# DakeQQ/Audio-Denoiser-ONNX

Measured on AMD Instinct MI355X. Metric: audio_seconds_per_second (GTCRN 16 kHz, batch=256 x 1 s chunks; RTF = 1/value), higher is better.
Workload: dtype f32; 1 GPU; GTCRN 16 kHz, batch=256 x 1 s chunks, fp32, int16 PCM in/out resident in HBM (BASELINE.json configs[1]); chunks_per_gpu=256, chunks_total=256, ranks=1, chunk_samples=16000, out_samples=15872, weights=seeded reference-architecture GTCRN (tests/golden/gtcrn_seed0.adew), stitch_all_gather=False

## Files before the change

audio_denoiser_onnx_amd/csrc/ade_device.h:

```cpp
#pragma once

#include "ade_internal.h"

namespace ade {
namespace dev {

__device__ __forceinline__ float fast_rcp(float x) { return __builtin_amdgcn_rcpf(x); }
__device__ __forceinline__ float fast_sqrt(float x) { return __builtin_amdgcn_sqrtf(x); }
__device__ __forceinline__ float fast_rsq(float x) { return __builtin_amdgcn_rsqf(x); }
__device__ __forceinline__ float sigmoid_f(float x) { return fast_rcp(1.0f + __expf(-x)); }
__device__ __forceinline__ float tanh_f(float x) {
    return 1.0f - 2.0f * fast_rcp(__expf(2.0f * x) + 1.0f);
}
__device__ __forceinline__ float prelu_f(float x, float a) { return x >= 0.0f ? x : a * x; }
__device__ __forceinline__ double shfl_xor_f64(double v, int mask) {
    union { double d; int i[2]; } u;
    u.d = v;
    u.i[0] = __shfl_xor(u.i[0], mask, 64);
    u.i[1] = __shfl_xor(u.i[1], mask, 64);
    return u.d;
}
__device__ __forceinline__ float prelu_sel(float a) { return a <= 1.0f ? __builtin_inff() : -__builtin_inff(); }
__device__ __forceinline__ float prelu_m(float x, float ax, float sel) { return __builtin_amdgcn_fmed3f(x, ax, sel); }

__device__ __forceinline__ void ld4(const float* p, float* v) {
    const float4 q = *reinterpret_cast<const float4*>(p);
    v[0] = q.x; v[1] = q.y; v[2] = q.z; v[3] = q.w;
}
__device__ __forceinline__ void ld8(const float* p, float* v) { ld4(p, v); ld4(p + 4, v + 4); }
__device__ __forceinline__ void ld16(const float* p, float* v) { ld8(p, v); ld8(p + 8, v + 8); }
__device__ __forceinline__ void st4(float* p, const float* v) {
    *reinterpret_cast<float4*>(p) = make_float4(v[0], v[1], v[2], v[3]);
}
__device__ __forceinline__ void st16(float* p, const float* v) { st4(p, v); st4(p + 4, v + 4); st4(p + 8, v + 8); st4(p + 12, v + 12); }

__device__ __forceinline__ void view_ld8_lo(const View& a, size_t pos, size_t frame, float* v) {
    ld8(a.x + pos * kCh, v);
    if (a.at) {
        float g[4];
        ld4(a.at + frame * 8, g);
#pragma unroll
        for (int i = 0; i < 4; ++i) v[2 * i] *= g[i];
    }
}
__device__ __forceinline__ void view_ld8_hi(const View& a, size_t pos, size_t frame, float* v) {
    ld8(a.x + pos * kCh + 8, v);
    if (a.at) {
        float g[4];
        ld4(a.at + frame * 8 + 4, g);
#pragma unroll
        for (int i = 0; i < 4; ++i) v[2 * i] *= g[i];
    }
}
__device__ __forceinline__ void view_ld16(const View& a, size_t pos, size_t frame, float* v) {
    view_ld8_lo(a, pos, frame, v);
    view_ld8_hi(a, pos, frame, v + 8);
}

template <int CTRL>
__device__ __forceinline__ float dpp_mov(float v) {
    return __int_as_float(__builtin_amdgcn_update_dpp(0, __float_as_int(v), CTRL, 0xF, 0xF, true));
}
template <int K> __device__ __forceinline__ float row_bcast(float v) { return dpp_mov<0x150 + K>(v); }
template <int K> __device__ __forceinline__ float quad_bcast(float v) { return dpp_mov<K * 0x55>(v); }
template <int N> __device__ __forceinline__ float row_ror(float v) { return dpp_mov<0x120 + N>(v); }
template <int N> __device__ __forceinline__ float quad_rot(float v) {
    return dpp_mov<((N) & 3) | (((N + 1) & 3) << 2) | (((N + 2) & 3) << 4) | (((N + 3) & 3) << 6)>(v);
}

struct Swapped { float a, b; };
__device__ __forceinline__ Swapped swap16(float v, float s) {
    const auto r = __builtin_amdgcn_permlane16_swap((unsigned)__float_as_int(v), (unsigned)__float_as_int(s), false, false);
    return Swapped{__int_as_float((int)r[0]), __int_as_float((int)r[1])};
}
__device__ __forceinline__ Swapped swap32(float v, float s) {
    const auto r = __builtin_amdgcn_permlane32_swap((unsigned)__float_as_int(v), (unsigned)__float_as_int(s), false, false);
    return Swapped{__int_as_float((int)r[0]), __int_as_float((int)r[1])};
}

template <int LANE> __device__ __forceinline__ float read_lane(float v) {
    return __int_as_float(__builtin_amdgcn_readlane(__float_as_int(v), LANE));
}
constexpr float kLog2e = 1.4426950408889634f;

#if defined(__clang__)
typedef float v4f __attribute__((ext_vector_type(4)));
#else
typedef float v4f __attribute__((vector_size(16)));
#endif
__device__ __forceinline__ v4f mfma16x16x4(float a, float b, v4f c) { return __builtin_amdgcn_mfma_f32_16x16x4f32(a, b, c, 0, 0, 0); }

#if defined(__clang__)
typedef float v2f __attribute__((ext_vector_type(2)));
#else
typedef float v2f __attribute__((vector_size(8)));
#endif
__device__ __forceinline__ v2f mk2(float a, float b) { v2f r; r[0] = a; r[1] = b; return r; }

#if defined(__has_attribute)
#if __has_attribute(address_space)
#define ADE_CONSTANT_AS __attribute__((address_space(4)))
#endif
#endif
#ifndef ADE_CONSTANT_AS
#define ADE_CONSTANT_AS
#endif
#if defined(__AMDGCN__)
#define ADE_KEEP_IN_LOOP(p) asm volatile("" : "+s"(p))
#else
#define ADE_KEEP_IN_LOOP(p) ((void)0)
#endif
#if defined(__AMDGCN__)
#define ADE_KEEP_AFTER(p, tok) asm volatile("" : "+s"(p), "+v"(tok))
#else
#define ADE_KEEP_AFTER(p, tok) ((void)0)
#endif
#if defined(__AMDGCN__)
#define ADE_SCALAR_COPY(dst, src) asm volatile("s_mov_b64 %0, %1" : "=s"(dst) : "s"(src))
#else
#define ADE_SCALAR_COPY(dst, src) ((dst) = (src))
#endif
#if defined(__AMDGCN__)
#define ADE_OPAQUE_V(x) asm volatile("" : "+v"(x))
#else
#define ADE_OPAQUE_V(x) ((void)0)
#endif
template <class T>
__device__ __forceinline__ T cload(const void ADE_CONSTANT_AS* p) {
    static_assert(sizeof(T) % 4 == 0, "dword-sized structs only");
    union U { T v; unsigned w[sizeof(T) / 4]; __device__ U() {} } u;
    const unsigned ADE_CONSTANT_AS* s = (const unsigned ADE_CONSTANT_AS*)p;
#pragma unroll
    for (size_t i = 0; i < sizeof(T) / 4; ++i) u.w[i] = s[i];
    return u.v;
}
typedef const float ADE_CONSTANT_AS* cfptr;
__device__ __forceinline__ cfptr cptr(const float* p) { return (cfptr)p; }

__device__ __forceinline__ void wave_sync() { __builtin_amdgcn_wave_barrier(); }
__device__ __forceinline__ float2 fcmul(float2 a, float2 b) { return make_float2(a.x * b.x - a.y * b.y, a.x * b.y + a.y * b.x); }
__device__ __forceinline__ void fradix4(float2* v) {
    const float2 a0 = make_float2(v[0].x + v[2].x, v[0].y + v[2].y);
    const float2 a1 = make_float2(v[0].x - v[2].x, v[0].y - v[2].y);
    const float2 a2 = make_float2(v[1].x + v[3].x, v[1].y + v[3].y);
    const float2 d = make_float2(v[1].x - v[3].x, v[1].y - v[3].y);
    const float2 a3 = make_float2(d.y, -d.x);
    v[0] = make_float2(a0.x + a2.x, a0.y + a2.y);
    v[1] = make_float2(a1.x + a3.x, a1.y + a3.y);
    v[2] = make_float2(a0.x - a2.x, a0.y - a2.y);
    v[3] = make_float2(a1.x - a3.x, a1.y - a3.y);
}
__device__ __forceinline__ void fft256_inplace(float2* v, float2* buf, int lane, const float2* __restrict__ tw256) {
    fradix4(v);
#pragma unroll
    for (int r = 0; r < 4; ++r) buf[4 * lane + r] = v[r];
    wave_sync();
#pragma unroll
    for (int pass = 1; pass < 4; ++pass) {
        const int Ns = 1 << (2 * pass);
        const int k = lane & (Ns - 1);
        const int tstride = 64 / Ns;
#pragma unroll
        for (int r = 0; r < 4; ++r) v[r] = buf[lane + 64 * r];
#pragma unroll
        for (int r = 1; r < 4; ++r) v[r] = fcmul(v[r], tw256[r * k * tstride]);
        fradix4(v);
        if (pass < 3) {
            wave_sync();
            const int j0 = ((lane - k) << 2) + k;
#pragma unroll
            for (int r = 0; r < 4; ++r) buf[j0 + r * Ns] = v[r];
            wave_sync();
        }
    }
}

__device__ __forceinline__ float4 keep4(bool ok, const float4& v) { return make_float4(ok ? v.x : 0.0f, ok ? v.y : 0.0f, ok ? v.z : 0.0f, ok ? v.w : 0.0f); }
__device__ __attribute__((aligned(16))) static float g_zero4[4] = {0.0f, 0.0f, 0.0f, 0.0f};
__device__ __forceinline__ float4 ld4_or_zero(bool ok, const float* p) { return *reinterpret_cast<const float4*>(ok ? p : g_zero4); }
__device__ __forceinline__ float4 pick4(bool first, const float4& a, const float4& b) {
    return make_float4(first ? a.x : b.x, first ? a.y : b.y, first ? a.z : b.z, first ? a.w : b.w);
}

#if defined(__AMDGCN__)
typedef unsigned ade_v4u __attribute__((ext_vector_type(4)));
__device__ __forceinline__ float4 xld4(const float* base, int float_off) {
    const __amdgpu_buffer_rsrc_t r = __builtin_amdgcn_make_buffer_rsrc(const_cast<float*>(base), 0, 0x7fffffff, 0x00020000);
    const ade_v4u v = __builtin_amdgcn_raw_buffer_load_b128(r, float_off * 4, 0, 16);
    return make_float4(__int_as_float((int)v.x), __int_as_float((int)v.y), __int_as_float((int)v.z), __int_as_float((int)v.w));
}
__device__ __forceinline__ void xst4(float* base, int float_off, const float4& v) {
    const __amdgpu_buffer_rsrc_t r = __builtin_amdgcn_make_buffer_rsrc(base, 0, 0x7fffffff, 0x00020000);
    ade_v4u u;
    u.x = (unsigned)__float_as_int(v.x); u.y = (unsigned)__float_as_int(v.y); u.z = (unsigned)__float_as_int(v.z); u.w = (unsigned)__float_as_int(v.w);
    __builtin_amdgcn_raw_buffer_store_b128(u, r, float_off * 4, 0, 16);
}
__device__ __forceinline__ float xld1(const float* p) { return __hip_atomic_load(p, __ATOMIC_RELAXED, __HIP_MEMORY_SCOPE_AGENT); }
__device__ __forceinline__ void xst1(float* p, float v) { __hip_atomic_store(p, v, __ATOMIC_RELAXED, __HIP_MEMORY_SCOPE_AGENT); }
__device__ __forceinline__ unsigned xflag_load(const unsigned* p) { return __hip_atomic_load(p, __ATOMIC_RELAXED, __HIP_MEMORY_SCOPE_AGENT); }
__device__ __forceinline__ void xflag_store(unsigned* p, unsigned v) { __hip_atomic_store(p, v, __ATOMIC_RELAXED, __HIP_MEMORY_SCOPE_AGENT); }
__device__ __forceinline__ void xdrain() { asm volatile("s_waitcnt vmcnt(0)" ::: "memory"); }
#else
__device__ __forceinline__ float4 xld4(const float* base, int float_off) { return *reinterpret_cast<const float4*>(base + float_off); }
__device__ __forceinline__ void xst4(float* base, int float_off, const float4& v) { *reinterpret_cast<float4*>(base + float_off) = v; }
__device__ __forceinline__ float xld1(const float* p) { return *p; }
__device__ __forceinline__ void xst1(float* p, float v) { *p = v; }
__device__ __forceinline__ unsigned xflag_load(const unsigned* p) { return *(const volatile unsigned*)p; }
__device__ __forceinline__ void xflag_store(unsigned* p, unsigned v) { *(volatile unsigned*)p = v; }
__device__ __forceinline__ void xdrain() {}
#endif
#if defined(__AMDGCN__)
__device__ __forceinline__ int xlimit() {
    const int ADE_CONSTANT_AS* p = (const int ADE_CONSTANT_AS*)__builtin_amdgcn_kernarg_segment_ptr();
    asm volatile("" : "+s"(p));
    return *p;
}
#else
__device__ __forceinline__ int xlimit() { return 20000000; }
#endif
__device__ __forceinline__ int xcode(int flag_index) { return (int)((blockIdx.x + 1u) << 4) | flag_index; }
__device__ __forceinline__ void xwait(unsigned* flag, int* err, int code) {
    if (xflag_load(flag) == 0u) {
        const long long t0 = wall_clock64();
        const int limit = xlimit();
        bool looked = false;
        do {
            __builtin_amdgcn_s_sleep(4);
            const long long dt = wall_clock64() - t0;
            if (dt > (limit >> 4) && !looked) {
                looked = true;
                if (*reinterpret_cast<volatile int*>(err) != 0) return;
            }
            if (dt > limit) {
                volatile int* const e = reinterpret_cast<volatile int*>(err);
                if (*e == 0) *e = code;
                return;
            }
        } while (xflag_load(flag) == 0u);
    }
    xflag_store(flag, 0u);
}

#if defined(__AMDGCN__)
__device__ __forceinline__ unsigned sys_load(const unsigned* p) { return __hip_atomic_load(p, __ATOMIC_RELAXED, __HIP_MEMORY_SCOPE_SYSTEM); }
__device__ __forceinline__ void sys_store(unsigned* p, unsigned v) { __hip_atomic_store(p, v, __ATOMIC_RELAXED, __HIP_MEMORY_SCOPE_SYSTEM); }
__device__ __forceinline__ void sys_acquire() { __builtin_amdgcn_fence(__ATOMIC_ACQUIRE, ""); }
__device__ __forceinline__ void sys_release() { __builtin_amdgcn_fence(__ATOMIC_RELEASE, ""); asm volatile("s_waitcnt vmcnt(0)" ::: "memory"); }
#else
__device__ __forceinline__ unsigned sys_load(const unsigned* p) { return *(const volatile unsigned*)p; }
__device__ __forceinline__ void sys_store(unsigned* p, unsigned v) { *(volatile unsigned*)p = v; }
__device__ __forceinline__ void sys_acquire() {}
__device__ __forceinline__ void sys_release() {}
#endif
__device__ __forceinline__ void wait_rows_in(const unsigned* ready, unsigned epoch, int* err, int code) {
    if (sys_load(ready) != epoch) {
        const long long t0 = wall_clock64();
        const int limit = xlimit();
        do {
            __builtin_amdgcn_s_sleep(8);
            if (wall_clock64() - t0 > limit) {
                volatile int* const e = reinterpret_cast<volatile int*>(err);
                if (*e == 0) *e = code;
                break;
            }
        } while (sys_load(ready) != epoch);
    }
    sys_acquire();
}
__device__ __forceinline__ void signal_rows_out(unsigned* count, unsigned* done, unsigned epoch, unsigned wgs) {
    sys_release();
#if defined(__AMDGCN__)
    const unsigned old = __hip_atomic_fetch_add(count, 1u, __ATOMIC_RELAXED, __HIP_MEMORY_SCOPE_AGENT);
#else
    const unsigned old = (*count)++;
#endif
    if (old + 1u == wgs) {
        xflag_store(count, 0u);
        sys_store(done, epoch);
    }
}

__device__ __forceinline__ void set_prio(int p) {
    if (p == 0) __builtin_amdgcn_s_setprio(0);
    else if (p == 1) __builtin_amdgcn_s_setprio(1);
    else if (p == 2) __builtin_amdgcn_s_setprio(2);
    else __builtin_amdgcn_s_setprio(3);
}

inline dim3 grid1(long long n, int per) { return dim3((unsigned)((n + per - 1) / per)); }

}
}
```

audio_denoiser_onnx_amd/csrc/ade_stage_net.h:

```cpp
#pragma once
#include "ade_device.h"

#include <type_traits>

#ifndef ADE_DP_INTER_MFMA
#define ADE_DP_INTER_MFMA 0
#endif

namespace ade {
namespace stage {

using namespace dev;


template <int NT, int TMAX, int WAVES_PER_SIMD>
struct Geo {
    static constexpr int kThreads = NT;
    static constexpr int kWavesPerSimd = WAVES_PER_SIMD;
    static constexpr int kTmax = TMAX;
    static constexpr int kPmax = TMAX * kFw;
    static constexpr int kPosPerThread = (kPmax + NT - 1) / NT;
    static constexpr int kTileF = NT / 64;
    static constexpr int kProdBase = ((TMAX * (kFw / 3) + 63) / 64) * 64;
    static constexpr bool kLean = NT < 512;
    static_assert(kPosPerThread == 3, "the conv phases are written for three positions per lane");
    static_assert(kProdBase < NT, "the history producers need a wavefront outside the conv lanes");
};
typedef Geo<1024, 64, 4> Geo0;
typedef Geo<512, 32, 4> Geo1;
typedef Geo<256, 16, 4> Geo2;

__device__ __forceinline__ float comp(const float4& v, int c) { return c == 0 ? v.x : (c == 1 ? v.y : (c == 2 ? v.z : v.w)); }

__device__ __forceinline__ void pl_ld8(const float* Xc, int P, int p, int q0, float* v) {
    ld4(Xc + ((size_t)q0 * P + p) * 4, v);
    ld4(Xc + ((size_t)(q0 + 1) * P + p) * 4, v + 4);
}
__device__ __forceinline__ void pl_ld16(const float* Xc, int P, int p, float* v) {
    pl_ld8(Xc, P, p, 0, v);
    pl_ld8(Xc, P, p, 2, v + 8);
}
__device__ __forceinline__ void pl_st16(float* Xc, int P, int p, const float* v) {
#pragma unroll
    for (int q = 0; q < 4; ++q) st4(Xc + ((size_t)q * P + p) * 4, v + 4 * q);
}

template <class G> constexpr size_t gt_smem_bytes() { return (size_t)4 * G::kPmax * 16 + 2 * G::kTmax * 8 * 4; }

#define ADE_REP16(M) M(0) M(1) M(2) M(3) M(4) M(5) M(6) M(7) M(8) M(9) M(10) M(11) M(12) M(13) M(14) M(15)

#define ADE_CLK(i) do { if (clk && chunk == 0 && threadIdx.x == 0) clk[i] = wall_clock64(); } while (0)
#define ADE_CLK_START() ((clk && chunk == 0 && threadIdx.x == 0) ? wall_clock64() : 0)
#define ADE_CLK_ACC(i) do { if (clk && chunk == 0 && threadIdx.x == 0) { const long long n_ = wall_clock64(); clk[i] += n_ - clk_prev; clk_prev = n_; } } while (0)

template <class G>
__device__ __forceinline__ void gtblock_stage(float4* smem, int chunk, const Seg& sg, int blk, const float* __restrict__ a, const float* __restrict__ skip,
                                              const GtConvW& w, float* __restrict__ out, long long* __restrict__ clk,
                                              bool x1_in_lds = false, bool next_x1 = false, const float* __restrict__ next_skip = nullptr, bool store_lo = true,
                                              bool next_full = false) {
    constexpr int kFusedThreads = G::kThreads, kTmaxFused = G::kTmax, kPmax = G::kPmax, kPosPerThread = G::kPosPerThread;
    float4* H = smem;
    float* zt = reinterpret_cast<float*>(smem + 4 * kPmax);
    float* at = zt + kTmaxFused * 8;
    float* GI = reinterpret_cast<float*>(smem + 2 * kPmax);
    float* HS = GI + kTmaxFused * 48;
    const int T = sg.nT;
    const int P = T * kFw;
    const int Ps = sg.T * kFw;
    int tid_ = threadIdx.x;
    if (kFusedThreads == 512 && sg.swap) tid_ ^= (tid_ & 256) >> 1;
    ADE_OPAQUE_V(tid_);
    const int tid = tid_;
    const size_t cbase = (size_t)chunk * kCh * Ps + (size_t)sg.t0 * kFw * 4;
    const float* ac = a + cbase;
    const float* sc = skip ? skip + cbase : nullptr;
    float* oc = out + cbase;
    const cfptr c_pw1_b = cptr(w.pw1_b), c_dw_b = cptr(w.dw_b), c_pw2_b = cptr(w.pw2_b);
    cfptr c_pw1, c_dw, c_pw2;
    ADE_SCALAR_COPY(c_pw1, cptr(w.pw1));
    ADE_SCALAR_COPY(c_dw, cptr(w.dw));
    ADE_SCALAR_COPY(c_pw2, cptr(w.pw2));
    const float pw1_slope = w.pw1_slope, dw_slope = w.dw_slope;
    const float pw1_sel = prelu_sel(pw1_slope), dw_sel = prelu_sel(dw_slope);
    const int dilation = w.dilation;
    ADE_CLK(0);

    if (!x1_in_lds) {
        constexpr int kIt = (kPmax + kFusedThreads - 1) / kFusedThreads;
        float x[kIt][8], y[kIt][8];
#pragma unroll
        for (int i = 0; i < kIt; ++i) {
            const int p = tid + i * kFusedThreads, pc = p < P ? p : P - 1;
            pl_ld8(ac, Ps, pc, 0, x[i]);
            if (sc) pl_ld8(sc, Ps, pc, 0, y[i]);
        }
#pragma unroll
        for (int i = 0; i < kIt; ++i) {
            const int p = tid + i * kFusedThreads;
            if (p >= P) break;
            if (sc) {
#pragma unroll
                for (int k = 0; k < 8; ++k) x[i][k] += y[i][k];
            }
            H[2 * kPmax + p] = make_float4(x[i][0], x[i][1], x[i][2], x[i][3]);
            H[3 * kPmax + p] = make_float4(x[i][4], x[i][5], x[i][6], x[i][7]);
        }
        __syncthreads();
    }
    constexpr int kWaves = kFusedThreads / 64;
    constexpr int kTiles = (kPmax / 16 + kWaves - 1) / kWaves;
    static_assert(kPmax % 16 == 0, "whole tiles");
    const int wave = __builtin_amdgcn_readfirstlane(tid >> 6);
    const int g = (tid >> 4) & 3, jn = tid & 15;
    const float* Hf = reinterpret_cast<const float*>(H);
    const char* const Hb = reinterpret_cast<const char*>(H);
    constexpr int kZ0 = 4 * kPmax * 16;
    constexpr int kPairs = (kTiles + 1) / 2;
    float4 hi[kPairs];
    {
        float wa[2][6];
#pragma unroll
        for (int kk = 0; kk < 6; ++kk) {
            wa[0][kk] = c_pw1[((4 * (kk & 1) + g) * 3 + (kk >> 1)) * 16 + jn];
            wa[1][kk] = c_pw1[((4 * (kk & 1) + g) * 3 + (kk >> 1)) * 16 + (jn ^ 8)];
        }
        v4f cb[2];
#pragma unroll
        for (int r = 0; r < 4; ++r) { cb[0][r] = c_pw1_b[4 * g + r]; cb[1][r] = c_pw1_b[(4 * g + r) ^ 8]; }
#pragma unroll
        for (int it = 0; it < kTiles; ++it) {
            const int od = it & 1;
            const int pu = (it * kWaves + wave) * 16 + jn, pos = pu < P ? pu : P - 1;
            const int f = pos - (pos / kFw) * kFw;
            const bool lok = f != 0, rok = f != kFw - 1;
            const char* xb = Hb + (pos * 4 + g) * 4;
            v4f d = cb[od];
#pragma unroll
            for (int kk = 0; kk < 6; ++kk) {
                const int o = kk >> 1;
                float x = *reinterpret_cast<const float*>(xb + ((2 + (kk & 1)) * kPmax + (o - 1)) * 16);
                if (o == 0) x = lok ? x : 0.0f;
                if (o == 2) x = rok ? x : 0.0f;
                d = mfma16x16x4(wa[od][kk], x, d);
            }
            const v2f d0 = mk2(d[0], d[1]), d1 = mk2(d[2], d[3]);
            const v2f a0 = d0 * mk2(pw1_slope, pw1_slope), a1 = d1 * mk2(pw1_slope, pw1_slope);
            const float4 r4 = make_float4(prelu_m(d0[0], a0[0], pw1_sel), prelu_m(d0[1], a0[1], pw1_sel),
                                          prelu_m(d1[0], a1[0], pw1_sel), prelu_m(d1[1], a1[1], pw1_sel));
            const bool now = (g < 2) != (od != 0);
            if (now && pu < P) H[(g & 1) * kPmax + pu] = r4;
            if (!od) {
                hi[it >> 1] = r4;
            } else {
                hi[it >> 1] = make_float4(now ? hi[it >> 1].x : r4.x, now ? hi[it >> 1].y : r4.y, now ? hi[it >> 1].z : r4.z, now ? hi[it >> 1].w : r4.w);
            }
        }
    }
    __syncthreads();
#pragma unroll
    for (int pr = 0; pr < kPairs; ++pr) {
        const int it = 2 * pr + (g < 2 ? 1 : 0);
        const int pu = (it * kWaves + wave) * 16 + jn;
        if (it < kTiles && pu < P) H[(2 + (g & 1)) * kPmax + pu] = hi[pr];
    }
    if (tid < 12) zt[tid] = 0.0f;
    if (sg.prev && tid == 0) xwait(sg.fi + kXFlagHist + blk, sg.err, xcode(kXFlagHist + blk));
    __syncthreads();
    ADE_CLK(1);

    float4 h1r[kPairs];
    {
        v2f wd[3][3][2];
#pragma unroll
        for (int kt = 0; kt < 3; ++kt)
#pragma unroll
            for (int kf = 0; kf < 3; ++kf) {
                const int o = kt * 48 + kf * 16 + 4 * g;
                wd[kt][kf][0] = mk2(c_dw[o], c_dw[o + 1]);
                wd[kt][kf][1] = mk2(c_dw[o + 2], c_dw[o + 3]);
            }
        const v2f db0 = mk2(c_dw_b[4 * g], c_dw_b[4 * g + 1]), db1 = mk2(c_dw_b[4 * g + 2], c_dw_b[4 * g + 3]);
        const int dstep = dilation * kFw * 16;
        const char* const zp = Hb + kZ0;
        auto dw_taps = [&](v2f& acc0, v2f& acc1, const int tj, const int f, const int prow, const int nkt) {
            const bool lok = f != 0, rok = f != kFw - 1;
            const char* const rb = Hb + ((g * kPmax + prow) * 16 - 16);
#pragma unroll
            for (int kt = 0; kt < 3; ++kt) {
                if (kt >= nkt) continue;
                const int src = tj - (2 - kt) * dilation;
                const bool tv = nkt == 3 ? (kt == 2 ? true : prow >= (2 - kt) * dilation * kFw) : (src >= 0 && src < T);
                const char* const row = tv ? rb - (2 - kt) * dstep : zp;
                const char* const la = lok ? row : zp;
                const char* const ra = rok ? row : zp;
                const float4 x0 = *reinterpret_cast<const float4*>(la);
                const float4 x1 = *reinterpret_cast<const float4*>(row + 16);
                const float4 x2 = *reinterpret_cast<const float4*>(ra + 32);
                acc0 += wd[kt][0][0] * mk2(x0.x, x0.y);
                acc1 += wd[kt][0][1] * mk2(x0.z, x0.w);
                acc0 += wd[kt][1][0] * mk2(x1.x, x1.y);
                acc1 += wd[kt][1][1] * mk2(x1.z, x1.w);
                acc0 += wd[kt][2][0] * mk2(x2.x, x2.y);
                acc1 += wd[kt][2][1] * mk2(x2.z, x2.w);
            }
        };
        float* const xhist_o = sg.xo + blk * kXHistFloats;
        const float* const xhist_i = sg.xi + blk * kXHistFloats;
        const int NP = 2 * dilation * kFw;
        if (sg.next) {
#pragma unroll 1
            for (int pt = wave; pt * 16 < NP; pt += kWaves) {
                const int pu = pt * 16 + jn, pn = pu < NP ? pu : NP - 1;
                const int tn = pn / kFw, f = pn - tn * kFw;
                const int j = tn + T;
                v2f acc0 = db0, acc1 = db1;
                if (sg.prev && j < 2 * dilation) {
                    const float4 v = xld4(xhist_i, (g * kXHistFrames * kFw + j * kFw + f) * 4);
                    acc0 = mk2(v.x, v.y);
                    acc1 = mk2(v.z, v.w);
                }
                dw_taps(acc0, acc1, j, f, pn + P, 2);
                if (pu < NP) xst4(xhist_o, (g * kXHistFrames * kFw + pn) * 4, make_float4(acc0[0], acc0[1], acc1[0], acc1[1]));
            }
            xdrain();
            __syncthreads();
            if (tid == 0) xflag_store(sg.fo + kXFlagHist + blk, 1u);
        }
        float wp[2][4];
#pragma unroll
        for (int r = 0; r < 4; ++r) {
            const float wv = c_pw2[(4 * g + r) * 8 + (jn & 7)];
            wp[0][r] = jn < 8 ? wv : 0.0f;
            wp[1][r] = jn < 8 ? 0.0f : wv;
        }
        v4f cb2;
#pragma unroll
        for (int r = 0; r < 4; ++r) cb2[r] = c_pw2_b[(4 * g + r) & 7];
        v4f d2 = cb2;
#pragma unroll
        for (int it = 0; it < kTiles; ++it) {
            const int pu = (it * kWaves + wave) * 16 + jn, pos = pu < P ? pu : P - 1;
            const int t = pos / kFw, f = pos - t * kFw;
            v2f acc0 = db0, acc1 = db1;
            if (sg.prev && (it * kWaves + wave) * 16 < NP) {
                const float4 v = xld4(xhist_i, (g * kXHistFrames * kFw + (pos < NP ? pos : NP - 1)) * 4);
                const bool head = pos < NP;
                acc0 = mk2(head ? v.x : db0[0], head ? v.y : db0[1]);
                acc1 = mk2(head ? v.z : db1[0], head ? v.w : db1[1]);
            }
            dw_taps(acc0, acc1, t, f, pos, 3);
            const v2f a0 = acc0 * mk2(dw_slope, dw_slope), a1 = acc1 * mk2(dw_slope, dw_slope);
            const float y[4] = {prelu_m(acc0[0], a0[0], dw_sel), prelu_m(acc0[1], a0[1], dw_sel),
                                prelu_m(acc1[0], a1[0], dw_sel), prelu_m(acc1[1], a1[1], dw_sel)};
            if (!(it & 1)) d2 = cb2;
#pragma unroll
            for (int r = 0; r < 4; ++r) d2 = mfma16x16x4(wp[it & 1][r], y[r], d2);
            if ((it & 1) || it == kTiles - 1) h1r[it >> 1] = make_float4(d2[0], d2[1], d2[2], d2[3]);
        }
    }
    __syncthreads();
    ADE_CLK(2);
#pragma unroll
    for (int pr = 0; pr < kPairs; ++pr) {
        const int it = 2 * pr + (g >> 1);
        const int pu = (it * kWaves + wave) * 16 + jn;
        if (it < kTiles && pu < P) H[(g & 1) * kPmax + pu] = h1r[pr];
    }
    __syncthreads();
    ADE_CLK(3);

    v2f wr_raw[8];
    float bh_raw = 0.0f;
    {
        const int j = tid & 15, row = (tid >> 4) & 3;
        const int gsel = (row & 1) ? 2 : (row >> 1);
        const float* pk = w.gru + j * 78 + 24 + gsel * 16;
#pragma unroll
        for (int m = 0; m < 8; ++m) wr_raw[m] = tid < 64 ? mk2(pk[2 * m], pk[2 * m + 1]) : mk2(0.0f, 0.0f);
        if (tid < 64) bh_raw = w.gru[j * 78 + 75 + gsel];
    }
    const float* nsc = (next_x1 && next_skip) ? next_skip + cbase : nullptr;
    float nsk[kPosPerThread][8];
    auto request_next_skip = [&]() {
#pragma unroll
        for (int i = 0; i < kPosPerThread; ++i) {
            const int p = tid + i * kFusedThreads;
            if (nsc && p < P) {
                pl_ld8(nsc, Ps, p, 0, nsk[i]);
            } else {
#pragma unroll
                for (int k = 0; k < 8; ++k) nsk[i][k] = 0.0f;
            }
        }
    };
    request_next_skip();
    {
        const int tr = tid >> 4, j = tid & 15;
        const int t = tr < T ? tr : T - 1;
        {
            float e[8] = {0.0f, 0.0f, 0.0f, 0.0f, 0.0f, 0.0f, 0.0f, 0.0f};
#pragma unroll
            for (int u = 0; u < 3; ++u) {
                const int f = j + 16 * u;
                if (f < kFw) {
                    const float4 a0 = H[t * kFw + f], a1 = H[kPmax + t * kFw + f];
                    e[0] += a0.x * a0.x; e[1] += a0.y * a0.y; e[2] += a0.z * a0.z; e[3] += a0.w * a0.w;
                    e[4] += a1.x * a1.x; e[5] += a1.y * a1.y; e[6] += a1.z * a1.z; e[7] += a1.w * a1.w;
                }
            }
#pragma unroll
            for (int c = 0; c < 8; ++c) {
                e[c] += row_ror<8>(e[c]);
                e[c] += row_ror<4>(e[c]);
                e[c] += row_ror<2>(e[c]);
                e[c] += row_ror<1>(e[c]);
                e[c] = e[c] * (1.0f / (float)kFw);
            }
            const float* pk = w.gru + j * 78;
#pragma unroll
            for (int g = 0; g < 3; ++g) {
                float sacc = pk[72 + g];
#pragma unroll
                for (int k = 0; k < 8; ++k) sacc += pk[g * 8 + k] * e[k];
                if (tr < T) GI[t * 48 + g * 16 + j] = sacc * (g == 2 ? 2.0f * kLog2e : -kLog2e);
            }
        }
    }
    if (sg.prev && tid == 0) xwait(sg.fi + kXFlagTra + blk, sg.err, xcode(kXFlagTra + blk));
    __syncthreads();
    ADE_CLK(4);
    ADE_CLK(5);
    if (tid >= 64) {
        constexpr int kLanes = kFusedThreads - 64, kIt = (kPmax + kLanes - 1) / kLanes;
        float by[kIt][8], y[kIt][8];
#pragma unroll
        for (int i = 0; i < kIt; ++i) {
            const int p = tid - 64 + i * kLanes, pc = p < P ? p : P - 1;
            pl_ld8(ac, Ps, pc, 2, by[i]);
            if (sc) pl_ld8(sc, Ps, pc, 2, y[i]);
        }
#pragma unroll
        for (int i = 0; i < kIt; ++i) {
            const int p = tid - 64 + i * kLanes;
            if (p >= P) break;
            if (sc) {
#pragma unroll
                for (int k = 0; k < 8; ++k) by[i][k] += y[i][k];
            }
            H[p] = make_float4(by[i][0], by[i][1], by[i][2], by[i][3]);
            H[kPmax + p] = make_float4(by[i][4], by[i][5], by[i][6], by[i][7]);
        }
    } else {
        const int j = tid & 15, row = tid >> 4;
        const int gsel = (row & 1) ? 2 : (row >> 1);
        const float sc = gsel == 2 ? 2.0f * kLog2e : -kLog2e;
        v2f wr[8];
#pragma unroll
        for (int m = 0; m < 8; ++m) wr[m] = wr_raw[m] * sc;
        const float bh = bh_raw * sc;
        int shb[16];
        float hv = 0.0f;
        if (sg.prev) hv = xld1(sg.xi + kXTraOff + blk * 16 + j);
#define ADE_RL(K) shb[K] = __builtin_amdgcn_readlane(__float_as_int(hv), K);
        ADE_REP16(ADE_RL)
#undef ADE_RL
        float gi = GI[gsel * 16 + j];
        float* hsp = row == 3 ? HS + j : GI + (tid & 63);
        const int hs_step = row == 3 ? 16 : 0;
        __builtin_amdgcn_s_setprio(3);
        for (int t = 0; t < T; ++t) {
            const int tn = t + 1 < T ? t + 1 : t;
            const float gnx = GI[tn * 48 + gsel * 16 + j];
#pragma unroll
            for (int k = 0; k < 16; ++k) ADE_KEEP_IN_LOOP(shb[k]);
            float sh[16];
#pragma unroll
            for (int k = 0; k < 16; ++k) sh[k] = __int_as_float(shb[k]);
            v2f a0 = mk2(bh, 0.0f), a1 = mk2(0.0f, 0.0f);
#pragma unroll
            for (int m = 0; m < 8; m += 2) {
                a0 += wr[m] * mk2(sh[2 * m], sh[2 * m + 1]);
                a1 += wr[m + 1] * mk2(sh[2 * m + 2], sh[2 * m + 3]);
            }
            const v2f a2 = a0 + a1;
            const float a = a2[0] + a2[1];
            const float e = __builtin_amdgcn_exp2f(gi + a);
            const float sg = fast_rcp(1.0f + e);
            const float X = swap16(e, sg).a;
            const float en = __builtin_amdgcn_exp2f(gi + X * a);
            const float n = 1.0f - 2.0f * fast_rcp(en + 1.0f);
            const float n3 = swap32(en, n).a;
            const float hc = n3 + X * (hv - n3);
            hv = hc;
#define ADE_RL(K) shb[K] = __builtin_amdgcn_readlane(__float_as_int(hc), 48 + K);
            ADE_REP16(ADE_RL)
#undef ADE_RL
            *hsp = hc;
            hsp += hs_step;
            gi = gnx;
        }
        set_prio(sg.base_prio);
        if (sg.next) {
            if (row == 3) xst1(sg.xo + kXTraOff + blk * 16 + j, hv);
            xdrain();
            if (tid == 48) xflag_store(sg.fo + kXFlagTra + blk, 1u);
        }
    }
    __syncthreads();
    ADE_CLK(6);
    for (int idx = tid; idx < T * 8; idx += kFusedThreads) {
        const int t = idx >> 3, c = idx & 7;
        const float* fr = w.fc + c * 17;
        float s = fr[16];
#pragma unroll
        for (int k = 0; k < 16; ++k) s += fr[k] * HS[t * 16 + k];
        at[idx] = sigmoid_f(s);
    }
    __syncthreads();
    ADE_CLK(7);
#pragma unroll
    for (int pr = 0; pr < kPairs; ++pr) {
        const int it = 2 * pr + (g >> 1);
        const int pu = (it * kWaves + wave) * 16 + jn;
        if (it < kTiles && pu < P) {
            const float4 gt = *reinterpret_cast<const float4*>(at + (pu / kFw) * 8 + 4 * (g & 1));
            H[(2 + (g & 1)) * kPmax + pu] = make_float4(h1r[pr].x * gt.x, h1r[pr].y * gt.y, h1r[pr].z * gt.z, h1r[pr].w * gt.w);
        }
    }
    __syncthreads();
    float n8[kPosPerThread][8];
#pragma unroll
    for (int i = 0; i < kPosPerThread; ++i) {
        const int p = tid + i * kFusedThreads;
        if (p < P) {
            const float4 b0 = H[p], b1 = H[kPmax + p], g0 = H[2 * kPmax + p], g1 = H[3 * kPmax + p];
            const float o[16] = {g0.x, b0.x, g0.y, b0.y, g0.z, b0.z, g0.w, b0.w, g1.x, b1.x, g1.y, b1.y, g1.z, b1.z, g1.w, b1.w};
            if (store_lo) {
                pl_st16(oc, Ps, p, o);
            } else {
                st4(oc + ((size_t)2 * Ps + p) * 4, o + 8);
                st4(oc + ((size_t)3 * Ps + p) * 4, o + 12);
            }
#pragma unroll
            for (int k = 0; k < 8; ++k) n8[i][k] = o[k] + nsk[i][k];
            if (next_full) {
#pragma unroll
                for (int q = 0; q < 4; ++q) H[q * kPmax + p] = make_float4(o[4 * q], o[4 * q + 1], o[4 * q + 2], o[4 * q + 3]);
            }
        }
    }
    if (next_x1) {
        __syncthreads();
#pragma unroll
        for (int i = 0; i < kPosPerThread; ++i) {
            const int p = tid + i * kFusedThreads;
            if (p < P) {
                H[2 * kPmax + p] = make_float4(n8[i][0], n8[i][1], n8[i][2], n8[i][3]);
                H[3 * kPmax + p] = make_float4(n8[i][4], n8[i][5], n8[i][6], n8[i][7]);
            }
        }
    }
    ADE_CLK(8);
}

template <class G> constexpr size_t dp_smem_bytes() { return (size_t)4 * G::kPmax * 16 + (size_t)2 * kFw * kCh * 4; }

template <class G, class EmitPos, class EmitOne>
__device__ __forceinline__ void fc_ln_rows(float4* R, const float* __restrict__ fc, const float* __restrict__ fc_b, const float* __restrict__ ln_w,
                                           const float* __restrict__ ln_b, int T, int P, int tid, const float* __restrict__ res, int Ps, EmitPos emit_pos, EmitOne emit_one) {
    constexpr int kFusedThreads = G::kThreads, kPmax = G::kPmax;
    static_assert(kFusedThreads / 16 >= G::kTmax, "one 16-lane row per frame");
    {
        constexpr int kWaves = kFusedThreads / 64, kTiles = (kPmax / 16 + kWaves - 1) / kWaves;
        int tq = tid;
        ADE_OPAQUE_V(tq);
        const int wave = __builtin_amdgcn_readfirstlane(tq >> 6), g = (tq >> 4) & 3, jn = tq & 15;
        float wa[4];
#pragma unroll
        for (int kk = 0; kk < 4; ++kk) wa[kk] = fc[(4 * g + kk) * 16 + jn];
        v4f cb;
#pragma unroll
        for (int r = 0; r < 4; ++r) cb[r] = fc_b[4 * g + r];
#pragma unroll
        for (int it = 0; it < kTiles; ++it) {
            const int pu = (it * kWaves + wave) * 16 + jn, pos = pu < P ? pu : P - 1;
            const float4 x = R[g * kPmax + pos];
            v4f d = cb;
            d = mfma16x16x4(wa[0], x.x, d);
            d = mfma16x16x4(wa[1], x.y, d);
            d = mfma16x16x4(wa[2], x.z, d);
            d = mfma16x16x4(wa[3], x.w, d);
            if (pu < P) R[g * kPmax + pu] = make_float4(d[0], d[1], d[2], d[3]);
        }
    }
    __syncthreads();
    int tq = tid;
    ADE_OPAQUE_V(tq);
    const int tr = tq >> 4, j = tq & 15;
    const bool live = tr < T;
    const int t = live ? tr : T - 1;
    const int p0 = t * kFw + j, p1 = p0 + 16, p2 = t * kFw + 32;
    float* Rf = reinterpret_cast<float*>(R);
    auto allreduce = [](float s) { s += row_ror<8>(s); s += row_ror<4>(s); s += row_ror<2>(s); s += row_ror<1>(s); return s; };
    float rs0[16], rs1[16];
    pl_ld16(res, Ps, p0, rs0);
    const float re = res[((size_t)(j >> 2) * Ps + p2) * 4 + (j & 3)];
    float v0[16], v1[16];
#pragma unroll
    for (int q = 0; q < 4; ++q) {
        const float4 a = R[q * kPmax + p0], b = R[q * kPmax + p1];
        v0[4 * q] = a.x; v0[4 * q + 1] = a.y; v0[4 * q + 2] = a.z; v0[4 * q + 3] = a.w;
        v1[4 * q] = b.x; v1[4 * q + 1] = b.y; v1[4 * q + 2] = b.z; v1[4 * q + 3] = b.w;
    }
    const float e = Rf[((size_t)(j >> 2) * kPmax + p2) * 4 + (j & 3)];
    float s = e;
#pragma unroll
    for (int c = 0; c < 16; ++c) s += v0[c] + v1[c];
    const float mean = allreduce(s) * (1.0f / (float)(kFw * kCh));
    const float de = e - mean;
    float q2 = de * de;
#pragma unroll
    for (int c = 0; c < 16; ++c) { const float a = v0[c] - mean, b = v1[c] - mean; q2 += a * a + b * b; }
    const float rstd = fast_rsq(allreduce(q2) * (1.0f / (float)(kFw * kCh)) + 1e-8f);
    {
        float gw[16], gb[16];
        ld16(ln_w + j * kCh, gw);
        ld16(ln_b + j * kCh, gb);
#pragma unroll
        for (int c = 0; c < 16; ++c) v0[c] = ((v0[c] - mean) * rstd * gw[c] + gb[c]) + rs0[c];
        if (live) emit_pos(p0, v0);
    }
    {
        float gw[16], gb[16];
        pl_ld16(res, Ps, p1, rs1);
        ld16(ln_w + (16 + j) * kCh, gw);
        ld16(ln_b + (16 + j) * kCh, gb);
#pragma unroll
        for (int c = 0; c < 16; ++c) v1[c] = ((v1[c] - mean) * rstd * gw[c] + gb[c]) + rs1[c];
        if (live) emit_pos(p1, v1);
    }
    {
        const float ye = (de * rstd * ln_w[32 * kCh + j] + ln_b[32 * kCh + j]) + re;
        if (live) emit_one(p2, j, ye);
    }
}

__device__ __forceinline__ float gru_gates(const v4f& d, float h) {
    const float r = fast_rcp(1.0f + __builtin_amdgcn_exp2f(d[0]));
    const float z = fast_rcp(1.0f + __builtin_amdgcn_exp2f(d[1]));
    const float n = 1.0f - 2.0f * fast_rcp(__builtin_amdgcn_exp2f(d[3] + r * d[2]) + 1.0f);
    return n + z * (h - n);
}

template <class G>
__device__ __forceinline__ void dpgrnn_stage(float4* smem, int chunk, const Seg& sg, int blk, const float* __restrict__ x, const DpW& w, float* __restrict__ out,
                                             long long* __restrict__ clk, bool next_x1 = false,
                                             const float* __restrict__ next_skip = nullptr, bool store_lo = true, bool x_in_lds = false, bool next_full = false) {
    constexpr int kFusedThreads = G::kThreads, kTmaxFused = G::kTmax, kPmax = G::kPmax, kPosPerThread = G::kPosPerThread;
    float4* R = smem;
    float* Rf = reinterpret_cast<float*>(smem);
    float* lnt = reinterpret_cast<float*>(smem + 4 * kPmax);
    const int T = sg.nT;
    const int P = T * kFw, Ps = sg.T * kFw;
    int tid_ = threadIdx.x;
    ADE_OPAQUE_V(tid_);
    const int tid = tid_;
    for (int i = tid; i < kFw * kCh; i += kFusedThreads) {
        lnt[i] = w.intra_ln_w[i];
        lnt[kFw * kCh + i] = w.intra_ln_b[i];
    }
    const size_t cbase = (size_t)chunk * kCh * Ps + (size_t)sg.t0 * kFw * 4;
    const float* xc = x + cbase;
    float* oc = out + cbase;

    ADE_CLK(16);
    {
        constexpr float kS = -kLog2e, kN = 2.0f * kLog2e;
        if (!x_in_lds) {
            float4 v[kPosPerThread][4];
#pragma unroll
            for (int i = 0; i < kPosPerThread; ++i) {
                const int p = tid + i * kFusedThreads, pc = p < P ? p : P - 1;
#pragma unroll
                for (int q = 0; q < 4; ++q) v[i][q] = *reinterpret_cast<const float4*>(xc + ((size_t)q * Ps + pc) * 4);
            }
#pragma unroll
            for (int i = 0; i < kPosPerThread; ++i) {
                const int p = tid + i * kFusedThreads;
                if (p < P) {
#pragma unroll
                    for (int q = 0; q < 4; ++q) R[q * kPmax + p] = v[i][q];
                }
            }
            __syncthreads();
        }
        const int wave = __builtin_amdgcn_readfirstlane(tid >> 6);
        const int g = (tid >> 4) & 3, j = tid & 15;
        const int grp = (wave >> 1) & 1, dir = wave & 1, t = (wave >> 2) * 16 + j;
        const bool live = t < T;
        const int tc = live ? t : T - 1;
        float ax0, ax1, ah;
        {
            const int c = j & 3;
            const float* pk = w.intra_gru + (grp * 8 + dir * 4 + (j >> 2)) * 42;
            const float sc_ = c < 2 ? kS : kN;
            const int gi = c == 3 ? 2 : c;
            ax0 = c == 2 ? 0.0f : pk[gi * 8 + g] * sc_;
            ax1 = c == 2 ? 0.0f : pk[gi * 8 + 4 + g] * sc_;
            ah = c == 3 ? 0.0f : pk[24 + c * 4 + g] * sc_;
        }
        v4f cb;
        {
            const float* pb = w.intra_gru + (grp * 8 + dir * 4 + g) * 42;
            cb[0] = (pb[36] + pb[39]) * kS;
            cb[1] = (pb[37] + pb[40]) * kS;
            cb[2] = pb[41] * kN;
            cb[3] = pb[38] * kN;
        }
        const float* const xr = Rf + ((size_t)(grp * 2) * kPmax + tc * kFw) * 4 + g;
        float hout[kFw];
        auto run = [&](auto dir_c) {
            constexpr int DIR = decltype(dir_c)::value;
            float h = 0.0f;
            __builtin_amdgcn_s_setprio(3);
            v4f dx;
            {
                constexpr int f0 = DIR ? kFw - 1 : 0;
                dx = mfma16x16x4(ax0, xr[f0 * 4], cb);
                dx = mfma16x16x4(ax1, xr[(kPmax + f0) * 4], dx);
            }
#pragma unroll
            for (int s = 0; s < kFw; ++s) {
                v4f d = mfma16x16x4(ah, h, dx);
                if (s + 1 < kFw) {
                    const int fn = DIR ? kFw - 2 - s : s + 1;
                    dx = mfma16x16x4(ax0, xr[fn * 4], cb);
                    dx = mfma16x16x4(ax1, xr[(kPmax + fn) * 4], dx);
                }
                h = gru_gates(d, h);
                hout[s] = h;
            }
            set_prio(sg.base_prio);
            __syncthreads();
            float* const hw = Rf + ((size_t)(grp * 2 + DIR) * kPmax + tc * kFw) * 4 + g;
            if (live) {
#pragma unroll
                for (int s = 0; s < kFw; ++s) hw[(DIR ? kFw - 1 - s : s) * 4] = hout[s];
            }
        };
        if (dir) run(std::integral_constant<int, 1>{});
        else run(std::integral_constant<int, 0>{});
    }
    __syncthreads();
    ADE_CLK(17);
    fc_ln_rows<G>(R, w.intra_fc, w.intra_fc_b, lnt, lnt + kFw * kCh, T, P, tid, xc, Ps,
        [&](int p, const float (&m)[16]) {
#pragma unroll
            for (int q = 0; q < 4; ++q) R[q * kPmax + p] = make_float4(m[4 * q], m[4 * q + 1], m[4 * q + 2], m[4 * q + 3]);
            pl_st16(oc, Ps, p, m);
        },
        [&](int p, int c, float m) {
            Rf[((size_t)(c >> 2) * kPmax + p) * 4 + (c & 3)] = m;
            oc[((size_t)(c >> 2) * Ps + p) * 4 + (c & 3)] = m;
        });
    if (sg.prev && tid == 0) xwait(sg.fi + kXFlagInter + blk, sg.err, xcode(kXFlagInter + blk));
    __syncthreads();
    for (int i = tid; i < kFw * kCh; i += kFusedThreads) {
        lnt[i] = w.inter_ln_w[i];
        lnt[kFw * kCh + i] = w.inter_ln_b[i];
    }
    ADE_CLK(18);
#if ADE_DP_INTER_MFMA
    {
        constexpr float kS = -kLog2e, kN = 2.0f * kLog2e;
        constexpr int kWaves = kFusedThreads / 64, kTilesC = 6;
        static_assert(kWaves % 2 == 0, "a wavefront's tiles share its group");
        const int wave = __builtin_amdgcn_readfirstlane(tid >> 6);
        const int g = (tid >> 4) & 3, j = tid & 15;
        const int grp = wave & 1;
        float ax[2][2], ah[2][2];
        v4f cb[2];
#pragma unroll
        for (int U = 0; U < 2; ++U) {
            const int c = j & 3;
            const float* pk = w.inter_gru + (grp * 8 + 4 * U + (j >> 2)) * 54;
            const float sc_ = c < 2 ? kS : kN;
            const int gi = c == 3 ? 2 : c;
#pragma unroll
            for (int kk = 0; kk < 2; ++kk) {
                ax[U][kk] = c == 2 ? 0.0f : pk[gi * 8 + 4 * kk + g] * sc_;
                ah[U][kk] = c == 3 ? 0.0f : pk[24 + c * 8 + 4 * kk + g] * sc_;
            }
            const float* pb = w.inter_gru + (grp * 8 + 4 * U + g) * 54;
            cb[U][0] = (pb[48] + pb[51]) * kS;
            cb[U][1] = (pb[49] + pb[52]) * kS;
            cb[U][2] = pb[53] * kN;
            cb[U][3] = pb[50] * kN;
        }
        auto run = [&](auto nt_c) {
            constexpr int NT = decltype(nt_c)::value;
            float h[NT][2];
            bool live[NT];
            float* xp[NT];
            float* xs[NT];
            v4f dx[NT][2];
#pragma unroll
            for (int c = 0; c < NT; ++c) {
                const int tile = wave + c * kWaves, f = (tile >> 1) * 16 + j;
                live[c] = f < kFw;
                const int fc = live[c] ? f : kFw - 1;
                xp[c] = Rf + ((size_t)(grp * 2) * kPmax + fc) * 4 + g;
                xs[c] = sg.xi + kXInterOff + blk * (kFw * 16) + fc * 16 + grp;
                h[c][0] = h[c][1] = 0.0f;
                if (sg.prev) {
                    h[c][0] = xld1(xs[c] + 2 * g);
                    h[c][1] = xld1(xs[c] + 2 * (4 + g));
                }
                const float x0 = xp[c][0], x1 = xp[c][kPmax * 4];
#pragma unroll
                for (int U = 0; U < 2; ++U) {
                    dx[c][U] = mfma16x16x4(ax[U][0], x0, cb[U]);
                    dx[c][U] = mfma16x16x4(ax[U][1], x1, dx[c][U]);
                }
            }
            __builtin_amdgcn_s_setprio(3);
            for (int t = 0; t < T; ++t) {
                const int tn = t + 1 < T ? 1 : 0;
#pragma unroll
                for (int c = 0; c < NT; ++c) {
// ... 168 lines not shown
```

Baseline: 764,300 audio-s/s.

## Remap GT-block MFMA tiles to frame-group-by-column layout with prefetched history loads

Reassigns each 16-lane MFMA tile from a flat contiguous position range to a fixed frequency column across 16 frames, so per-lane division and modulo by the frame width and most edge masks become compile-time or per-wave constants. Depthwise taps now use precomputed row offsets, and the predecessor-history head loads are software-pipelined several tiles ahead through bounds-checked buffer loads. The zero strip is widened so that out-of-range slots read zeros. The cost is more complex indexing, extra registers for the prefetched values, and a risk of layout or edge-handling bugs.

```diff
diff --git a/audio_denoiser_onnx_amd/csrc/ade_device.h b/audio_denoiser_onnx_amd/csrc/ade_device.h
--- a/audio_denoiser_onnx_amd/csrc/ade_device.h
+++ b/audio_denoiser_onnx_amd/csrc/ade_device.h
@@ -189,6 +189,11 @@
     const ade_v4u v = __builtin_amdgcn_raw_buffer_load_b128(r, float_off * 4, 0, 16);
     return make_float4(__int_as_float((int)v.x), __int_as_float((int)v.y), __int_as_float((int)v.z), __int_as_float((int)v.w));
 }
+__device__ __forceinline__ float4 xld4_within(const float* base, int float_off, int bytes) {
+    const __amdgpu_buffer_rsrc_t r = __builtin_amdgcn_make_buffer_rsrc(const_cast<float*>(base), 0, bytes, 0x00020000);
+    const ade_v4u v = __builtin_amdgcn_raw_buffer_load_b128(r, float_off * 4, 0, 16);
+    return make_float4(__int_as_float((int)v.x), __int_as_float((int)v.y), __int_as_float((int)v.z), __int_as_float((int)v.w));
+}
 __device__ __forceinline__ void xst4(float* base, int float_off, const float4& v) {
     const __amdgpu_buffer_rsrc_t r = __builtin_amdgcn_make_buffer_rsrc(base, 0, 0x7fffffff, 0x00020000);
     ade_v4u u;
@@ -202,6 +207,9 @@
 __device__ __forceinline__ void xdrain() { asm volatile("s_waitcnt vmcnt(0)" ::: "memory"); }
 #else
 __device__ __forceinline__ float4 xld4(const float* base, int float_off) { return *reinterpret_cast<const float4*>(base + float_off); }
+__device__ __forceinline__ float4 xld4_within(const float* base, int float_off, int bytes) {
+    return float_off >= 0 && float_off * 4 + 16 <= bytes ? *reinterpret_cast<const float4*>(base + float_off) : make_float4(0.0f, 0.0f, 0.0f, 0.0f);
+}
 __device__ __forceinline__ void xst4(float* base, int float_off, const float4& v) { *reinterpret_cast<float4*>(base + float_off) = v; }
 __device__ __forceinline__ float xld1(const float* p) { return *p; }
 __device__ __forceinline__ void xst1(float* p, float v) { *p = v; }
diff --git a/audio_denoiser_onnx_amd/csrc/ade_stage_net.h b/audio_denoiser_onnx_amd/csrc/ade_stage_net.h
--- a/audio_denoiser_onnx_amd/csrc/ade_stage_net.h
+++ b/audio_denoiser_onnx_amd/csrc/ade_stage_net.h
@@ -1,5 +1,9 @@
 #pragma once
 #include "ade_device.h"
+
+#ifndef ADE_HEAD_AHEAD
+#define ADE_HEAD_AHEAD 4
+#endif
 
 #include <type_traits>
 
@@ -47,7 +51,15 @@
 
 template <class G> constexpr size_t gt_smem_bytes() { return (size_t)4 * G::kPmax * 16 + 2 * G::kTmax * 8 * 4; }
 
-#define ADE_REP16(M) M(0) M(1) M(2) M(3) M(4) M(5) M(6) M(7) M(8) M(9) M(10) M(11) M(12) M(13) M(14) M(15)
+constexpr bool tile_may_be_column(int it, int waves, int groups, int col) {
+    for (int w = 0; w < waves; ++w) {
+        const int k = it * waves + w, fg = k / kFw < groups ? k / kFw : groups - 1;
+        if (k - fg * kFw == col) return true;
+    }
+    return false;
+}
+
+#define ADE_REP16(M)M(0) M(1) M(2) M(3) M(4) M(5) M(6) M(7) M(8) M(9) M(10) M(11) M(12) M(13) M(14) M(15)
 
 #define ADE_CLK(i) do { if (clk && chunk == 0 && threadIdx.x == 0) clk[i] = wall_clock64(); } while (0)
 #define ADE_CLK_START() ((clk && chunk == 0 && threadIdx.x == 0) ? wall_clock64() : 0)
@@ -108,13 +120,30 @@
         __syncthreads();
     }
     constexpr int kWaves = kFusedThreads / 64;
-    constexpr int kTiles = (kPmax / 16 + kWaves - 1) / kWaves;
-    static_assert(kPmax % 16 == 0, "whole tiles");
+    constexpr int kTileCount = kPmax / 16, kFg = kTmaxFused / 16;
+    constexpr int kTiles = (kTileCount + kWaves - 1) / kWaves;
+    static_assert(kTmaxFused % 16 == 0, "whole frame groups");
     const int wave = __builtin_amdgcn_readfirstlane(tid >> 6);
     const int g = (tid >> 4) & 3, jn = tid & 15;
-    const float* Hf = reinterpret_cast<const float*>(H);
+    struct Tile { int fg, f; bool ok; };
+    auto tile_at = [&](const int it) {
+        const int k = it * kWaves + wave;
+        int fg = 0;
+        if (kFg > 1) { fg = k / kFw; fg = fg < kFg ? fg : kFg - 1; }
+        return Tile{fg, k - fg * kFw, k < kTileCount};
+    };
+    const int f0 = tile_at(0).f;
+    struct Slot { int pos, frame; bool live; };
+    auto pair_slot = [&](const int pr, const bool odd, const int jn) {
+        const Tile te = tile_at(2 * pr), to = tile_at(2 * pr + 1);
+        const int fg = odd ? to.fg : te.fg, f = odd ? to.f : te.f;
+        const int frame = fg * 16 + jn;
+        return Slot{frame * kFw + f, frame, (odd ? to.ok : te.ok) && frame < T};
+    };
     const char* const Hb = reinterpret_cast<const char*>(H);
-    constexpr int kZ0 = 4 * kPmax * 16;
+    constexpr int kZ0 = 4 * kPmax * 16, kZeroBytes = (kFw + 2) * 16;
+    static_assert(kZeroBytes / 4 <= kFusedThreads, "one store per lane fills the zero strip");
+    static_assert(kZeroBytes + (kTiles * kWaves - kTileCount) * 16 <= 2 * kTmaxFused * 8 * 4, "the zero strip, and what the slots past the last tile read behind it, fits zt | at");
     constexpr int kPairs = (kTiles + 1) / 2;
     float4 hi[kPairs];
     {
@@ -130,17 +159,18 @@
 #pragma unroll
         for (int it = 0; it < kTiles; ++it) {
             const int od = it & 1;
-            const int pu = (it * kWaves + wave) * 16 + jn, pos = pu < P ? pu : P - 1;
-            const int f = pos - (pos / kFw) * kFw;
-            const bool lok = f != 0, rok = f != kFw - 1;
-            const char* xb = Hb + (pos * 4 + g) * 4;
+            const Tile tl = tile_at(it);
+            const bool medge0 = tile_may_be_column(it, kWaves, kFg, 0), medge2 = tile_may_be_column(it, kWaves, kFg, kFw - 1);
+            const int frame = tl.fg * 16 + jn, fc = frame < T ? frame : T - 1;
+            const char* xb = Hb + ((fc * kFw + f0) * 4 + g) * 4;
+            const int df = tl.f - f0;
             v4f d = cb[od];
 #pragma unroll
             for (int kk = 0; kk < 6; ++kk) {
                 const int o = kk >> 1;
-                float x = *reinterpret_cast<const float*>(xb + ((2 + (kk & 1)) * kPmax + (o - 1)) * 16);
-                if (o == 0) x = lok ? x : 0.0f;
-                if (o == 2) x = rok ? x : 0.0f;
+                float x = *reinterpret_cast<const float*>(xb + ((2 + (kk & 1)) * kPmax + df + (o - 1)) * 16);
+                if (o == 0 && medge0) x = tl.f == 0 ? 0.0f : x;
+                if (o == 2 && medge2) x = tl.f == kFw - 1 ? 0.0f : x;
                 d = mfma16x16x4(wa[od][kk], x, d);
             }
             const v2f d0 = mk2(d[0], d[1]), d1 = mk2(d[2], d[3]);
@@ -148,7 +178,7 @@
             const float4 r4 = make_float4(prelu_m(d0[0], a0[0], pw1_sel), prelu_m(d0[1], a0[1], pw1_sel),
                                           prelu_m(d1[0], a1[0], pw1_sel), prelu_m(d1[1], a1[1], pw1_sel));
             const bool now = (g < 2) != (od != 0);
-            if (now && pu < P) H[(g & 1) * kPmax + pu] = r4;
+            if (now && tl.ok && frame < T) H[(g & 1) * kPmax + frame * kFw + f0 + df] = r4;
             if (!od) {
                 hi[it >> 1] = r4;
             } else {
@@ -157,13 +187,14 @@
         }
     }
     __syncthreads();
+    int jq = tid & 15;
+    ADE_OPAQUE_V(jq);
 #pragma unroll
     for (int pr = 0; pr < kPairs; ++pr) {
-        const int it = 2 * pr + (g < 2 ? 1 : 0);
-        const int pu = (it * kWaves + wave) * 16 + jn;
-        if (it < kTiles && pu < P) H[(2 + (g & 1)) * kPmax + pu] = hi[pr];
-    }
-    if (tid < 12) zt[tid] = 0.0f;
+        const Slot s = pair_slot(pr, g < 2, jq);
+        if (s.live) H[(2 + (g & 1)) * kPmax + s.pos] = hi[pr];
+    }
+    if (tid < kZeroBytes / 4) zt[tid] = 0.0f;
     if (sg.prev && tid == 0) xwait(sg.fi + kXFlagHist + blk, sg.err, xcode(kXFlagHist + blk));
     __syncthreads();
     ADE_CLK(1);
@@ -181,32 +212,44 @@
             }
         const v2f db0 = mk2(c_dw_b[4 * g], c_dw_b[4 * g + 1]), db1 = mk2(c_dw_b[4 * g + 2], c_dw_b[4 * g + 3]);
         const int dstep = dilation * kFw * 16;
+        auto dw_tap = [&](v2f& acc0, v2f& acc1, const int kt, const char* la, const char* ca, const char* ra) {
+            const float4 x0 = *reinterpret_cast<const float4*>(la);
+            const float4 x1 = *reinterpret_cast<const float4*>(ca);
+            const float4 x2 = *reinterpret_cast<const float4*>(ra);
+            acc0 += wd[kt][0][0] * mk2(x0.x, x0.y);
+            acc1 += wd[kt][0][1] * mk2(x0.z, x0.w);
+            acc0 += wd[kt][1][0] * mk2(x1.x, x1.y);
+            acc1 += wd[kt][1][1] * mk2(x1.z, x1.w);
+            acc0 += wd[kt][2][0] * mk2(x2.x, x2.y);
+            acc1 += wd[kt][2][1] * mk2(x2.z, x2.w);
+        };
         const char* const zp = Hb + kZ0;
-        auto dw_taps = [&](v2f& acc0, v2f& acc1, const int tj, const int f, const int prow, const int nkt) {
+        auto dw_hist_taps = [&](v2f& acc0, v2f& acc1, const int tj, const int f, const int prow) {
             const bool lok = f != 0, rok = f != kFw - 1;
             const char* const rb = Hb + ((g * kPmax + prow) * 16 - 16);
 #pragma unroll
-            for (int kt = 0; kt < 3; ++kt) {
-                if (kt >= nkt) continue;
+            for (int kt = 0; kt < 2; ++kt) {
                 const int src = tj - (2 - kt) * dilation;
-                const bool tv = nkt == 3 ? (kt == 2 ? true : prow >= (2 - kt) * dilation * kFw) : (src >= 0 && src < T);
-                const char* const row = tv ? rb - (2 - kt) * dstep : zp;
-                const char* const la = lok ? row : zp;
-                const char* const ra = rok ? row : zp;
-                const float4 x0 = *reinterpret_cast<const float4*>(la);
-                const float4 x1 = *reinterpret_cast<const float4*>(row + 16);
-                const float4 x2 = *reinterpret_cast<const float4*>(ra + 32);
-                acc0 += wd[kt][0][0] * mk2(x0.x, x0.y);
-                acc1 += wd[kt][0][1] * mk2(x0.z, x0.w);
-                acc0 += wd[kt][1][0] * mk2(x1.x, x1.y);
-                acc1 += wd[kt][1][1] * mk2(x1.z, x1.w);
-                acc0 += wd[kt][2][0] * mk2(x2.x, x2.y);
-                acc1 += wd[kt][2][1] * mk2(x2.z, x2.w);
+                const char* const row = (src >= 0 && src < T) ? rb - (2 - kt) * dstep : zp;
+                dw_tap(acc0, acc1, kt, lok ? row : zp, row + 16, (rok ? row : zp) + 32);
             }
         };
         float* const xhist_o = sg.xo + blk * kXHistFloats;
         const float* const xhist_i = sg.xi + blk * kXHistFloats;
         const int NP = 2 * dilation * kFw;
+        static_assert(kXHistFrames <= 16, "the frames that continue the predecessor's sums are all in frame group 0");
+        const int own = (g * kPmax + jn * kFw + f0) * 16 - 16, zown = kZ0 + f0 * 16;
+        int rowb[3];
+#pragma unroll
+        for (int kt = 0; kt < 3; ++kt) rowb[kt] = (jn < T && jn >= (2 - kt) * dilation) ? own - (2 - kt) * dstep : zown;
+        const bool head = sg.prev && jn < 2 * dilation;
+        const int hoff = (g * kXHistFrames * kFw + (head ? jn : 0) * kFw + f0) * 4;
+        constexpr int kHeadAhead = ADE_HEAD_AHEAD;
+        const int hbytes = sg.prev ? kXHistFloats * 4 : 0;
+        auto head_load = [&](const int it) { return xld4_within(xhist_i, hoff + (tile_at(it).f - f0) * 4, hbytes); };
+        float4 hv[kTiles];
+#pragma unroll
+        for (int it = 0; it < kHeadAhead && it < kTiles; ++it) hv[it] = head_load(it);
         if (sg.next) {
 #pragma unroll 1
             for (int pt = wave; pt * 16 < NP; pt += kWaves) {
@@ -219,7 +262,7 @@
                     acc0 = mk2(v.x, v.y);
                     acc1 = mk2(v.z, v.w);
                 }
-                dw_taps(acc0, acc1, j, f, pn + P, 2);
+                dw_hist_taps(acc0, acc1, j, f, pn + P);
                 if (pu < NP) xst4(xhist_o, (g * kXHistFrames * kFw + pn) * 4, make_float4(acc0[0], acc0[1], acc1[0], acc1[1]));
             }
             xdrain();
@@ -239,16 +282,27 @@
         v4f d2 = cb2;
 #pragma unroll
         for (int it = 0; it < kTiles; ++it) {
-            const int pu = (it * kWaves + wave) * 16 + jn, pos = pu < P ? pu : P - 1;
-            const int t = pos / kFw, f = pos - t * kFw;
+            const Tile tl = tile_at(it);
+            const bool medge0 = tile_may_be_column(it, kWaves, kFg, 0), medge2 = tile_may_be_column(it, kWaves, kFg, kFw - 1);
+            const int df = tl.f - f0;
             v2f acc0 = db0, acc1 = db1;
-            if (sg.prev && (it * kWaves + wave) * 16 < NP) {
-                const float4 v = xld4(xhist_i, (g * kXHistFrames * kFw + (pos < NP ? pos : NP - 1)) * 4);
-                const bool head = pos < NP;
-                acc0 = mk2(head ? v.x : db0[0], head ? v.y : db0[1]);
-                acc1 = mk2(head ? v.z : db1[0], head ? v.w : db1[1]);
-            }
-            dw_taps(acc0, acc1, t, f, pos, 3);
+            {
+                if (it + kHeadAhead < kTiles) hv[it + kHeadAhead] = head_load(it + kHeadAhead);
+                const float4 v = hv[it];
+                const bool hd = kFg > 1 ? head && tl.fg == 0 : head;
+                acc0 = mk2(hd ? v.x : db0[0], hd ? v.y : db0[1]);
+                acc1 = mk2(hd ? v.z : db1[0], hd ? v.w : db1[1]);
+            }
+#pragma unroll
+            for (int kt = 0; kt < 3; ++kt) {
+                int rb = rowb[kt];
+                if (kFg > 1 && tl.fg != 0) rb = jn < T - tl.fg * 16 ? own + tl.fg * (16 * kFw * 16) - (2 - kt) * dstep : zown;
+                const char* const row = Hb + rb + df * 16;
+                const char *la = row, *ra = row + 32;
+                if (medge0 && tl.f == 0) la = zp;
+                if (medge2 && tl.f == kFw - 1) ra = zp;
+                dw_tap(acc0, acc1, kt, la, row + 16, ra);
+            }
             const v2f a0 = acc0 * mk2(dw_slope, dw_slope), a1 = acc1 * mk2(dw_slope, dw_slope);
             const float y[4] = {prelu_m(acc0[0], a0[0], dw_sel), prelu_m(acc0[1], a0[1], dw_sel),
                                 prelu_m(acc1[0], a1[0], dw_sel), prelu_m(acc1[1], a1[1], dw_sel)};
@@ -260,11 +314,12 @@
     }
     __syncthreads();
     ADE_CLK(2);
+    jq = tid & 15;
+    ADE_OPAQUE_V(jq);
 #pragma unroll
     for (int pr = 0; pr < kPairs; ++pr) {
-        const int it = 2 * pr + (g >> 1);
-        const int pu = (it * kWaves + wave) * 16 + jn;
-        if (it < kTiles && pu < P) H[(g & 1) * kPmax + pu] = h1r[pr];
+        const Slot s = pair_slot(pr, g >= 2, jq);
+        if (s.live) H[(g & 1) * kPmax + s.pos] = h1r[pr];
     }
     __syncthreads();
     ADE_CLK(3);
@@ -418,13 +473,14 @@
     }
     __syncthreads();
     ADE_CLK(7);
+    jq = tid & 15;
+    ADE_OPAQUE_V(jq);
 #pragma unroll
     for (int pr = 0; pr < kPairs; ++pr) {
-        const int it = 2 * pr + (g >> 1);
-        const int pu = (it * kWaves + wave) * 16 + jn;
-        if (it < kTiles && pu < P) {
-            const float4 gt = *reinterpret_cast<const float4*>(at + (pu / kFw) * 8 + 4 * (g & 1));
-            H[(2 + (g & 1)) * kPmax + pu] = make_float4(h1r[pr].x * gt.x, h1r[pr].y * gt.y, h1r[pr].z * gt.z, h1r[pr].w * gt.w);
+        const Slot s = pair_slot(pr, g >= 2, jq);
+        if (s.live) {
+            const float4 gt = *reinterpret_cast<const float4*>(at + s.frame * 8 + 4 * (g & 1));
+            H[(2 + (g & 1)) * kPmax + s.pos] = make_float4(h1r[pr].x * gt.x, h1r[pr].y * gt.y, h1r[pr].z * gt.z, h1r[pr].w * gt.w);
         }
     }
     __syncthreads();
```

New measurement: 765,000 audio-s/s (median of 6 runs). About the same (+0.1%).
